# byuccl/coast

Hardware: NVIDIA H100
Metric: protected-kernel throughput (MB/s voted output), sha256 TMR (higher is better)
Workload: dtype u32

## Files before the change

coast_b200/csrc/xmr_aes128.cuh:

```cuda
#pragma once
#include "xmr_common.cuh"
#include "aes_tables.inc"

namespace xmr {

constexpr int AES_THREADS = XMR_AES_THREADS, AES_WARPS = XMR_AES_WARPS;
constexpr uint32_t AES_TAB01 = XMR_AES_TAB01, AES_TAB23 = XMR_AES_TAB23, AES_SIS = XMR_AES_SIS;
static_assert(AES_TAB01 + 256u * 64u * 4u <= AES_TAB23 && AES_TAB23 + 256u * 64u * 4u <= xmr_aes_smem(false) &&
              AES_SIS + 256u * 32u * 4u <= xmr_aes_smem(true), "the tables fit the launch's shared memory");
template <int NC> struct AesGeom {
    static constexpr int J = (int)xmr_aes_blocks_per_lane(NC);
    static constexpr int TROWS = AES_WARPS * Lanes<NC>::kUnitsPerWarp * J;
    static_assert(TROWS == xmr_aes_tile_rows(NC), "the host's tile");
};

constexpr int AES_STAGES = 3;
template <int TILE_ROWS>
struct AesRing {
    static constexpr int LOADS = (int)xmr_ring_loads(TILE_ROWS);
    static constexpr int BOX_ROWS = TILE_ROWS / LOADS;
    static constexpr uint32_t TILE_BYTES = (uint32_t)TILE_ROWS * 16u;
    static constexpr uint32_t STAGE_STRIDE = xmr_ring_stride(TILE_ROWS, 16u);
    static constexpr uint32_t SMEM_BYTES = xmr_ring_smem(AES_STAGES, TILE_ROWS, 16u, 128u);
    static_assert(2 * AES_STAGES * sizeof(uint64_t) <= 128u, "full and empty barriers fit behind the tiles");
    uint8_t* tiles; uint64_t* full; uint64_t* empty; const CUtensorMap* tmap; uint32_t pack_shift;
    __device__ __forceinline__ void init(uint8_t* smem, const CUtensorMap* map, uint32_t row_pack_shift) {
        tiles = smem; tmap = map; pack_shift = row_pack_shift;
        full = reinterpret_cast<uint64_t*>(smem + AES_STAGES * STAGE_STRIDE);
        empty = full + AES_STAGES;
        if (threadIdx.x == 0) {
            tma_prefetch_desc(map);
#pragma unroll
            for (int s = 0; s < AES_STAGES; ++s) { mbar_init(&full[s], 1); mbar_init(&empty[s], AES_WARPS); }
            fence_barrier_init();
        }
        __syncthreads();
    }
    __device__ __forceinline__ void issue(uint32_t it, uint32_t tile) {
        const uint32_t stage = it % AES_STAGES;
        mbar_arrive_expect_tx(&full[stage], TILE_BYTES);
#pragma unroll
        for (int l = 0; l < LOADS; ++l)
            tma_load_2d(tiles + stage * STAGE_STRIDE + l * BOX_ROWS * 16, tmap, &full[stage], 0, (int)((tile * TILE_ROWS + l * BOX_ROWS) >> pack_shift));
    }
    __device__ __forceinline__ const uint8_t* wait_full(uint32_t it) {
        mbar_wait(&full[it % AES_STAGES], (it / AES_STAGES) & 1u);
        return tiles + (it % AES_STAGES) * STAGE_STRIDE;
    }
    __device__ __forceinline__ void release(uint32_t it, int lane) {
        __syncwarp();
        if (lane == 0) asm volatile("mbarrier.arrive.shared::cta.b64 _, [%0];" ::"r"(smem_u32(&empty[it % AES_STAGES])) : "memory");
    }
    __device__ __forceinline__ void wait_empty(uint32_t it) {
        mbar_wait(&empty[it % AES_STAGES], (it / AES_STAGES) & 1u);
    }
};

__device__ __forceinline__ uint32_t lds32(uint32_t saddr) { uint32_t v; asm volatile("ld.shared.u32 %0, [%1];" : "=r"(v) : "r"(saddr)); return v; }
template <int K> __device__ __forceinline__ uint32_t tab(uint32_t lb, uint32_t t) { return lds32(__byte_perm(t, lb, 0x7604u | (K << 4))); }
template <int K> __device__ __forceinline__ uint32_t tab_half(uint32_t lb2x, uint32_t t) { return lds32(__byte_perm(t, lb2x, 0x7604u | (K << 4)) >> 1); }

__device__ __forceinline__ uint32_t xtime4(uint32_t w) { return ((w & 0x7F7F7F7Fu) << 1) ^ (((w >> 7) & 0x01010101u) * 0x1Bu); }
__device__ __forceinline__ uint32_t mix_column(uint32_t w) {
    const uint32_t r1 = __byte_perm(w, 0u, 0x0321u), r2 = __byte_perm(w, 0u, 0x1032u), r3 = __byte_perm(w, 0u, 0x2103u);
    return xtime4(w ^ r1) ^ r1 ^ r2 ^ r3;
}
__device__ __forceinline__ uint32_t inv_mix_column(uint32_t w) {
    const uint32_t v = w ^ __byte_perm(w, 0u, 0x1032u);
    return mix_column(w ^ xtime4(xtime4(v)));
}

struct AesLaneBases { uint32_t lb0, lb1, lb2, lb3, sis2x; };

template <bool DEC> __device__ __forceinline__ uint32_t sub_rot_word(const AesLaneBases& L, uint32_t w) {
    if (DEC) {
        const uint32_t a = tab_half<1>(L.sis2x, w), b = tab_half<2>(L.sis2x, w), c = tab_half<3>(L.sis2x, w), d = tab_half<0>(L.sis2x, w);
        return __byte_perm(__byte_perm(a, b, 0x0051u), __byte_perm(c, d, 0x0051u), 0x5410u);
    }
    return (tab<1>(L.lb2, w) & 0x000000FFu) | (tab<2>(L.lb0, w) & 0x0000FF00u) | (tab<3>(L.lb0, w) & 0x00FF0000u) | (tab<0>(L.lb1, w) & 0xFF000000u);
}
template <bool DEC> __device__ __forceinline__ void key_next(const AesLaneBases& L, uint32_t (&k)[4], int rd) {
    k[0] ^= sub_rot_word<DEC>(L, k[3]) ^ (uint32_t)XMR_AES_RCON[rd];
    k[1] ^= k[0]; k[2] ^= k[1]; k[3] ^= k[2];
}
template <bool DEC> __device__ __forceinline__ void key_prev(const AesLaneBases& L, uint32_t (&k)[4], int rd) {
    k[3] ^= k[2]; k[2] ^= k[1]; k[1] ^= k[0];
    k[0] ^= sub_rot_word<DEC>(L, k[3]) ^ (uint32_t)XMR_AES_RCON[rd];
}

template <bool DEC, bool LAST>
__device__ __forceinline__ void aes_round_cols(const AesLaneBases& L, const uint32_t (&t)[4], uint32_t (&n)[4]) {
    if (!DEC) {
        if (!LAST) {
#pragma unroll
            for (int c = 0; c < 4; ++c)
                n[c] = tab<0>(L.lb0, t[c]) ^ tab<1>(L.lb1, t[(c + 1) & 3]) ^ tab<2>(L.lb2, t[(c + 2) & 3]) ^ tab<3>(L.lb3, t[(c + 3) & 3]);
        } else {
#pragma unroll
            for (int c = 0; c < 4; ++c)
                n[c] = (tab<0>(L.lb2, t[c]) & 0x000000FFu) | (tab<1>(L.lb0, t[(c + 1) & 3]) & 0x0000FF00u) |
                       (tab<2>(L.lb0, t[(c + 2) & 3]) & 0x00FF0000u) | (tab<3>(L.lb1, t[(c + 3) & 3]) & 0xFF000000u);
        }
    } else {
        if (!LAST) {
#pragma unroll
            for (int c = 0; c < 4; ++c)
                n[c] = tab<0>(L.lb0, t[c]) ^ tab<1>(L.lb1, t[(c + 3) & 3]) ^ tab<2>(L.lb2, t[(c + 2) & 3]) ^ tab<3>(L.lb3, t[(c + 1) & 3]);
        } else {
#pragma unroll
            for (int c = 0; c < 4; ++c) {
                const uint32_t a = tab_half<0>(L.sis2x, t[c]), b = tab_half<1>(L.sis2x, t[(c + 3) & 3]);
                const uint32_t d = tab_half<2>(L.sis2x, t[(c + 2) & 3]), e = tab_half<3>(L.sis2x, t[(c + 1) & 3]);
                n[c] = __byte_perm(__byte_perm(a, b, 0x0040u), __byte_perm(d, e, 0x0040u), 0x5410u);
            }
        }
    }
}

template <int NC>
__device__ __forceinline__ void aes_vote_store(const uint32_t (&c)[4], uint8_t* out, unsigned long long local,
                                               unsigned long long gunit, bool valid, int lane, uint32_t flags, Tally& tally) {
    const bool majority = flags & COAST_F_MAJORITY_VOTER;
    uint32_t o[4], bad = 0;
#pragma unroll
    for (int i = 0; i < 4; ++i) { Voted v = vote_u32<NC, 1>(c[i], majority); o[i] = v.vote; bad += v.bad; }
    if (valid && Lanes<NC>::voter(lane)) {
        *reinterpret_cast<uint4*>(out + local * 16ull) = make_uint4(o[0], o[1], o[2], o[3]);
        tally.unit_exit<NC>(bad, 16u, flags, gunit);
    }
}

template <int J, bool DEC, bool PERKEY, bool HOOKS, bool ROLLED = false>
__device__ __forceinline__ void aes_rounds(const AesLaneBases& L, uint32_t (&s)[J][4], uint32_t (&k)[PERKEY ? J : 1][4], const uint32_t (&rk)[PERKEY ? 4 : 44],
                                           const uint32_t (&fbit)[J], const int (&frd)[J], const int (&fcol)[J]) {
    static_assert(!ROLLED || PERKEY, "a rolled round loop cannot index the register-resident round keys");
#pragma unroll (ROLLED ? 1 : 10)
    for (int rd = 0; rd < 10; ++rd) {
#pragma unroll
        for (int j = 0; j < J; ++j) {
            uint32_t n[4];
            if (rd < 9) aes_round_cols<DEC, false>(L, s[j], n); else aes_round_cols<DEC, true>(L, s[j], n);
            if (HOOKS) {
                uint32_t hit = frd[j] == rd ? fbit[j] : 0u;
                if (DEC && rd < 9) hit = inv_mix_column(hit);
#pragma unroll
                for (int c = 0; c < 4; ++c) n[c] ^= fcol[j] == c ? hit : 0u;
            }
            if (PERKEY) {
                if (!DEC) {
                    key_next<false>(L, k[j], rd);
#pragma unroll
                    for (int c = 0; c < 4; ++c) s[j][c] = n[c] ^ k[j][c];
                } else {
                    key_prev<true>(L, k[j], 9 - rd);
#pragma unroll
                    for (int c = 0; c < 4; ++c) s[j][c] = n[c] ^ (rd < 9 ? inv_mix_column(k[j][c]) : k[j][c]);
                }
            } else {
#pragma unroll
                for (int c = 0; c < 4; ++c) s[j][c] = n[c] ^ rk[4 * (rd + 1) + c];
            }
        }
    }
}

template <int J, bool DEC>
__device__ __forceinline__ void aes_rounds_hooked(const AesLaneBases& L, uint32_t (&s)[J][4], uint32_t rk_saddr,
                                               const uint32_t (&fbit)[J], const int (&frd)[J], const int (&fcol)[J]) {
#pragma unroll 1
    for (int rd = 0; rd < 10; ++rd) {
        uint32_t kr[4];
#pragma unroll
        for (int c = 0; c < 4; ++c) kr[c] = lds32(rk_saddr + 16u * (uint32_t)(rd + 1) + 4u * c);
#pragma unroll
        for (int j = 0; j < J; ++j) {
            uint32_t n[4];
            if (rd < 9) aes_round_cols<DEC, false>(L, s[j], n); else aes_round_cols<DEC, true>(L, s[j], n);
            uint32_t hit = frd[j] == rd ? fbit[j] : 0u;
            if (DEC && rd < 9) hit = inv_mix_column(hit);
#pragma unroll
            for (int c = 0; c < 4; ++c) s[j][c] = n[c] ^ (fcol[j] == c ? hit : 0u) ^ kr[c];
        }
    }
}

template <bool DEC>
__device__ __forceinline__ void aes_build_tables(uint8_t* smem_raw, uint32_t win, int tid) {
    uint32_t* t01 = reinterpret_cast<uint32_t*>(smem_raw + (AES_TAB01 - win));
    uint32_t* t23 = reinterpret_cast<uint32_t*>(smem_raw + (AES_TAB23 - win));
    for (int i = tid; i < 256 * 64; i += AES_THREADS) {
        uint32_t v;
        if (!DEC) v = XMR_AES_TE0[i >> 6];
        else v = inv_mix_column((uint32_t)XMR_AES_RSBOX[i >> 6]);
        const bool hi = (i & 32) != 0;
        t01[i] = hi ? __byte_perm(v, 0u, 0x2103u) : v;
        t23[i] = hi ? __byte_perm(v, 0u, 0x0321u) : __byte_perm(v, 0u, 0x1032u);
    }
    if (DEC) {
        uint32_t* sis = reinterpret_cast<uint32_t*>(smem_raw + (AES_SIS - win));
        for (int i = tid; i < 256 * 32; i += AES_THREADS) {
            const uint32_t is = XMR_AES_RSBOX[i >> 5], sb = XMR_AES_SBOX[i >> 5];
            sis[i] = is | (sb << 8) | (is << 16) | (sb << 24);
        }
    }
}
__device__ __forceinline__ AesLaneBases aes_lane_bases(int lane) {
    AesLaneBases L;
    L.lb0 = AES_TAB01 + 4u * lane; L.lb1 = AES_TAB01 + 128u + 4u * lane;
    L.lb2 = AES_TAB23 + 4u * lane; L.lb3 = AES_TAB23 + 128u + 4u * lane;
// ... 309 lines not shown
```

coast_b200/csrc/xmr_common.cuh:

```cuda
#pragma once
#include <cuda.h>
#include <cuda_runtime.h>
#include <stdint.h>
#include "../../include/coast_rt.h"
#include "xmr_args.h"
#include "xmr_geom.h"

namespace xmr {

struct u4 { uint32_t x, y, z, w; };

__device__ __forceinline__ u4 philox4x32_10(uint32_t c0, uint32_t c1, uint32_t c2, uint32_t c3, uint32_t k0, uint32_t k1) {
#pragma unroll
    for (int r = 0; r < 10; ++r) {
        uint32_t hi0 = __umulhi(0xD2511F53u, c0), lo0 = 0xD2511F53u * c0;
        uint32_t hi1 = __umulhi(0xCD9E8D57u, c2), lo1 = 0xCD9E8D57u * c2;
        uint32_t n0 = hi1 ^ c1 ^ k0, n2 = hi0 ^ c3 ^ k1;
        c0 = n0; c1 = lo1; c2 = n2; c3 = lo0;
        k0 += 0x9E3779B9u; k1 += 0xBB67AE85u;
    }
    return u4{c0, c1, c2, c3};
}

struct Fault { bool active; uint32_t replica, site, bit; };
// ... 72 lines not shown
    uint32_t e01 = eq_mask<EB>(x, r1), e02 = eq_mask<EB>(x, r2);
    v.vote = majority ? ((x & r1) | (x & r2) | (r1 & r2)) : ((x & e01) | (r2 & ~e01));
    v.bad = __popc(~(e01 & e02)) / (8 * EB);
    return v;
}

template <int NC>
__device__ __forceinline__ Voted vote_f32(float x, bool majority) {
    uint32_t xb = __float_as_uint(x);
    Voted v{xb, 0u};
    if (NC == 1) return v;
    float r1 = __shfl_down_sync(0xFFFFFFFFu, x, 1);
    if (NC == 2) { v.bad = (x == r1) ? 0u : 1u; return v; }
    float r2 = __shfl_down_sync(0xFFFFFFFFu, x, 2);
    bool c01 = (x == r1), c02 = (x == r2);
    uint32_t b1 = __float_as_uint(r1), b2 = __float_as_uint(r2);
    v.vote = majority ? ((xb & b1) | (xb & b2) | (b1 & b2)) : (c01 ? xb : b2);
    v.bad = (c01 && c02) ? 0u : 1u;
    return v;
}

template <int NC>
__device__ __forceinline__ uint32_t store_vote(uint32_t& x, int lane, bool majority) {
    if (NC == 1) return 0u;
    const int base = Lanes<NC>::unit(lane) * NC;
    const uint32_t r0 = __shfl_sync(0xFFFFFFFFu, x, base), r1 = __shfl_sync(0xFFFFFFFFu, x, base + 1);
    if (NC == 2) return r0 != r1 ? 1u : 0u;
    const uint32_t r2 = __shfl_sync(0xFFFFFFFFu, x, base + 2);
    const bool c01 = r0 == r1, c02 = r0 == r2;
    x = majority ? ((r0 & r1) | (r0 & r2) | (r1 & r2)) : (c01 ? r0 : r2);
    return (c01 && c02) ? 0u : 1u;
}

template <int NC>
__device__ __forceinline__ uint32_t store_vote_bytes(uint32_t& x, uint32_t nb, int lane, bool majority) {
    if (NC == 1 || nb == 0u) return 0u;
    const uint32_t live = 0xFFFFFFFFu << (8u * (4u - nb));
    const int base = Lanes<NC>::unit(lane) * NC;
    const uint32_t r0 = __shfl_sync(0xFFFFFFFFu, x, base), r1 = __shfl_sync(0xFFFFFFFFu, x, base + 1);
    const uint32_t e01 = __vcmpeq4(r0, r1);
    if (NC == 2) return __popc(~e01 & live) >> 3;
    const uint32_t r2 = __shfl_sync(0xFFFFFFFFu, x, base + 2);
    const uint32_t e02 = __vcmpeq4(r0, r2);
    x = majority ? ((r0 & r1) | (r0 & r2) | (r1 & r2)) : ((r0 & e01) | (r2 & ~e01));
    return __popc(~(e01 & e02) & live) >> 3;
}

struct Tally {
    uint32_t errors = 0, dwc = 0, syncs = 0, injected = 0;
    unsigned long long first = ~0ull;
    unsigned char* status = nullptr;
    unsigned long long base = 0;
    __device__ __forceinline__ Tally() {}
    __device__ __forceinline__ explicit Tally(const xmr_args& a) : status(a.status), base(a.unit_base) {}
    template <int NC> __device__ __forceinline__ void unit_exit(uint32_t bad, uint32_t nvotes, uint32_t flags, unsigned long long gunit) {
        if (NC == 3) {
            if (flags & COAST_F_COUNT_ERRORS) {
                errors += bad;
                if (flags & COAST_F_COUNT_SYNCS) syncs += nvotes;
            }
        } else if (NC == 2) {
            dwc += bad ? 1u : 0u;
        }
        if (NC > 1 && bad && gunit < first) first = gunit;
        if (status) status[gunit - base] = (unsigned char)(NC > 1 ? (bad > 255u ? 255u : bad) : 0u);
    }
    __device__ __forceinline__ void flush(unsigned long long* ctr) {
        uint32_t e = __reduce_add_sync(0xFFFFFFFFu, errors);
        uint32_t d = __reduce_add_sync(0xFFFFFFFFu, dwc);
        uint32_t s = __reduce_add_sync(0xFFFFFFFFu, syncs);
        uint32_t j = __reduce_add_sync(0xFFFFFFFFu, injected);
        uint32_t fhi = __reduce_min_sync(0xFFFFFFFFu, (uint32_t)(first >> 32));
        uint32_t flo = __reduce_min_sync(0xFFFFFFFFu, (uint32_t)(first >> 32) == fhi ? (uint32_t)first : 0xFFFFFFFFu);
        if ((threadIdx.x & 31) == 0) {
            if (e) atomicAdd_system(ctr + XMR_CTR_ERRORS, (unsigned long long)e);
            if (d) atomicAdd_system(ctr + XMR_CTR_DWC, (unsigned long long)d);
            if (s) atomicAdd_system(ctr + XMR_CTR_SYNCS, (unsigned long long)s);
            if (j) atomicAdd_system(ctr + XMR_CTR_INJECTED, (unsigned long long)j);
            unsigned long long f = ((unsigned long long)fhi << 32) | flo;
            if (f != ~0ull) atomicMin_system(ctr + XMR_CTR_FIRST, f);
        }
    }
};

__device__ __forceinline__ uint32_t smem_u32(const void* p) { return (uint32_t)__cvta_generic_to_shared(p); }

__device__ __forceinline__ void mbar_init(uint64_t* bar, uint32_t count) {
    asm volatile("mbarrier.init.shared::cta.b64 [%0], %1;" ::"r"(smem_u32(bar)), "r"(count));
}
__device__ __forceinline__ void fence_barrier_init() { asm volatile("fence.mbarrier_init.release.cluster;" ::: "memory"); }
__device__ __forceinline__ void fence_proxy_async() { asm volatile("fence.proxy.async.shared::cta;" ::: "memory"); }
__device__ __forceinline__ void mbar_arrive_expect_tx(uint64_t* bar, uint32_t bytes) {
    asm volatile("mbarrier.arrive.expect_tx.shared::cta.b64 _, [%0], %1;" ::"r"(smem_u32(bar)), "r"(bytes) : "memory");
}
__device__ __forceinline__ void mbar_wait(uint64_t* bar, uint32_t parity) {
    asm volatile(
        "{\n\t.reg .pred p;\n\t"
        "WAIT_%=:\n\t"
        "mbarrier.try_wait.parity.shared::cta.b64 p, [%0], %1;\n\t"
        "@p bra DONE_%=;\n\t"
        "bra WAIT_%=;\n\t"
        "DONE_%=:\n\t}" ::"r"(smem_u32(bar)), "r"(parity) : "memory");
}
__device__ __forceinline__ void tma_load_2d(void* smem_dst, const CUtensorMap* map, uint64_t* bar, int c0, int c1) {
    asm volatile(
        "cp.async.bulk.tensor.2d.shared::cluster.global.tile.mbarrier::complete_tx::bytes [%0], [%1, {%3, %4}], [%2];"
        ::"r"(smem_u32(smem_dst)), "l"(map), "r"(smem_u32(bar)), "r"(c0), "r"(c1) : "memory");
}
__device__ __forceinline__ void tma_prefetch_desc(const CUtensorMap* map) {
    asm volatile("prefetch.tensormap [%0];" ::"l"(map) : "memory");
}

template <int TILE_ROWS, int ROW_BYTES>
struct TileRing {
    static constexpr int LOADS = (int)xmr_ring_loads(TILE_ROWS);
    static constexpr int BOX_ROWS = TILE_ROWS / LOADS;
    static_assert(TILE_ROWS % LOADS == 0 && BOX_ROWS <= 256, "tile must split into equal TMA boxes");
    static constexpr uint32_t TILE_BYTES = (uint32_t)TILE_ROWS * ROW_BYTES;
    static constexpr uint32_t STAGE_STRIDE = xmr_ring_stride(TILE_ROWS, ROW_BYTES);
    static constexpr uint32_t SMEM_BYTES = xmr_ring_smem(XMR_STAGES, TILE_ROWS, ROW_BYTES, XMR_RING_TAIL);
    static_assert(XMR_STAGES * sizeof(uint64_t) <= XMR_RING_TAIL, "the full barriers fit behind the tiles");
    uint8_t* tiles;
    uint64_t* full;
    const CUtensorMap* tmap;
    uint32_t pack_shift = 0;
    __device__ __forceinline__ void init(uint8_t* smem, const CUtensorMap* map, uint32_t row_pack_shift = 0) {
        pack_shift = row_pack_shift;
        tiles = smem;
        full = reinterpret_cast<uint64_t*>(smem + XMR_STAGES * STAGE_STRIDE);
        tmap = map;
        if (threadIdx.x == 0) {
            tma_prefetch_desc(map);
#pragma unroll
            for (int s = 0; s < XMR_STAGES; ++s) mbar_init(&full[s], 1);
            fence_barrier_init();
        }
        __syncthreads();
    }
    __device__ __forceinline__ void issue(uint32_t stage, uint32_t tile) {
        if (threadIdx.x == 0) {
            mbar_arrive_expect_tx(&full[stage], TILE_BYTES);
#pragma unroll
            for (int l = 0; l < LOADS; ++l)
                tma_load_2d(tiles + stage * STAGE_STRIDE + l * BOX_ROWS * ROW_BYTES, tmap, &full[stage], 0,
                            (int)((tile * TILE_ROWS + l * BOX_ROWS) >> pack_shift));
        }
    }
    __device__ __forceinline__ const uint8_t* wait(uint32_t it) {
        mbar_wait(&full[it & 1u], (it >> 1) & 1u);
        return tiles + (it & 1u) * STAGE_STRIDE;
    }
};

}
```

coast_b200/csrc/xmr_geom.h:

```cpp
#ifndef XMR_GEOM_H_
#define XMR_GEOM_H_

#ifdef __CUDACC__
#define XMR_GEOM_FN static constexpr __host__ __device__ inline
#else
#define XMR_GEOM_FN static inline
#endif

XMR_GEOM_FN unsigned xmr_align(unsigned x, unsigned a) { return (x + a - 1u) & ~(a - 1u); }
XMR_GEOM_FN unsigned xmr_ring_stride(unsigned tile_rows, unsigned row_bytes) { return xmr_align(tile_rows * row_bytes, 1024u); }
XMR_GEOM_FN unsigned xmr_ring_smem(unsigned stages, unsigned tile_rows, unsigned row_bytes, unsigned tail) {
    return stages * xmr_ring_stride(tile_rows, row_bytes) + tail;
}
XMR_GEOM_FN unsigned xmr_ring_loads(unsigned tile_rows) {
    unsigned l = (tile_rows + 255u) / 256u;
    while (tile_rows % l) ++l;
    return l;
}
XMR_GEOM_FN unsigned xmr_units_per_warp(unsigned nc) { return 32u / nc; }

#define XMR_CTA_THREADS 256
#define XMR_WARPS       8
#define XMR_STAGES      2
#define XMR_RING_TAIL   64u
XMR_GEOM_FN unsigned xmr_sha_tile_rows(unsigned nc) { return XMR_WARPS * xmr_units_per_warp(nc); }
XMR_GEOM_FN unsigned xmr_sha_smem(unsigned nc) { return xmr_ring_smem(XMR_STAGES, xmr_sha_tile_rows(nc), 64u, XMR_RING_TAIL); }

#define XMR_SHA_SEG_THREADS    384
#define XMR_SHA_SEG_TILE_ROWS  128u
#define XMR_SHA_SEG_EXCH_BYTES (2u * 4u * 2u * 8u * 32u * 4u)
XMR_GEOM_FN unsigned xmr_sha_seg_exch_offset(void) {
    return xmr_align(xmr_ring_smem(XMR_STAGES, XMR_SHA_SEG_TILE_ROWS, 64u, XMR_RING_TAIL), 128u);
}
XMR_GEOM_FN unsigned xmr_sha_seg_smem(void) { return xmr_sha_seg_exch_offset() + XMR_SHA_SEG_EXCH_BYTES; }

#define XMR_CRC_TAB  0x10000u
#define XMR_CRC_RING 0x20000u
XMR_GEOM_FN unsigned xmr_crc_threads(unsigned nc) { return nc == 1u ? 768u : 1024u; }
XMR_GEOM_FN unsigned xmr_crc_tile_rows(unsigned nc) { return xmr_crc_threads(nc) / 32u * xmr_units_per_warp(nc); }
XMR_GEOM_FN unsigned xmr_crc_smem(unsigned nc) { return XMR_CRC_RING + xmr_ring_smem(XMR_STAGES, xmr_crc_tile_rows(nc), 64u, XMR_RING_TAIL); }

#define XMR_AES_THREADS 512
#define XMR_AES_WARPS   16
#define XMR_AES_TAB01   0x10000u
#define XMR_AES_TAB23   0x20000u
#define XMR_AES_SIS     0x30000u
XMR_GEOM_FN unsigned xmr_aes_blocks_per_lane(unsigned nc) { return nc == 1u ? 2u : 4u; }
XMR_GEOM_FN unsigned xmr_aes_tile_rows(unsigned nc) { return XMR_AES_WARPS * xmr_units_per_warp(nc) * xmr_aes_blocks_per_lane(nc); }
XMR_GEOM_FN unsigned xmr_aes_smem(int dec) { return dec ? XMR_AES_SIS + 0x8000u : XMR_AES_SIS; }

#define XMR_MMT_BM 64u
#define XMR_MMT_BN 128u
#define XMR_MMT_BK 16u
#define XMR_MMT_VT 128u
#define XMR_MMT_SMEM (64u * 1024u)
XMR_GEOM_FN unsigned xmr_mmt_threads(unsigned nc) { return nc * XMR_MMT_VT; }

#define XMR_WG_THREADS      384
#define XMR_WG_BM           128u
#define XMR_WG_SMEM_TAIL    (1024u + 256u)
#define XMR_PREPASS_THREADS 256
#define XMR_GEMM_BK 32u
XMR_GEOM_FN unsigned xmr_gemm_bn(int wide) { return wide ? 256u : 128u; }
XMR_GEOM_FN unsigned xmr_gemm_stages(int wide) { return wide ? 4u : 6u; }
XMR_GEOM_FN unsigned xmr_gemm_b_box(int pair) { return pair ? 64u : 128u; }
XMR_GEOM_FN unsigned xmr_gemm_smem(int wide) {
    return xmr_gemm_stages(wide) * (XMR_WG_BM * XMR_GEMM_BK * 4u + XMR_GEMM_BK * xmr_gemm_bn(wide) * 4u) + XMR_WG_SMEM_TAIL;
}
#define XMR_GEMM_BF16_BK    64u
#define XMR_GEMM_BF16_B_BOX 64u
#define XMR_MMTC_BK     128u
#define XMR_MMTC_STAGES 2u
XMR_GEOM_FN unsigned xmr_mmtc_bn(unsigned nc) { return nc == 1u ? 64u : 32u; }
XMR_GEOM_FN unsigned xmr_mmtc_smem(unsigned nc) {
    return XMR_MMTC_STAGES * (4u * XMR_WG_BM * XMR_MMTC_BK + 4u * xmr_mmtc_bn(nc) * XMR_MMTC_BK) + XMR_WG_SMEM_TAIL;
}

#define XMR_QSORT_THREADS 128

#define XMR_RAGGED_BUCKETS      1024u
#define XMR_RAGGED_HDR          64u
#define XMR_RAGGED_PERM         (XMR_RAGGED_HDR + 4u * XMR_RAGGED_BUCKETS)
#define XMR_RAGGED_SCAN_THREADS 1024
#define XMR_RAGGED_COST_CRC     0u
#define XMR_RAGGED_COST_SHA     1u
#define XMR_RAGGED_COST_QSORT   2u
XMR_GEOM_FN unsigned long long xmr_ragged_scratch(unsigned long long n_units) { return XMR_RAGGED_PERM + 4ull * n_units; }
XMR_GEOM_FN unsigned long long xmr_ragged_slots(unsigned long long n_units) { return (xmr_ragged_scratch(n_units) + 127ull) & ~127ull; }

#define XMR_MM_GRP_SCAN_THREADS 1024
#define XMR_MM_GRP_TILES        128u
#define XMR_MM_GRP_MAX          (1u << 20)
XMR_GEOM_FN unsigned long long xmr_mm_grp_bytes(unsigned long long groups) { return XMR_MM_GRP_TILES + 4ull * (groups + 1ull); }

#endif
```

coast_b200/csrc/xmr_sha256.cuh:

```cuda
#pragma once
#include "xmr_common.cuh"

namespace xmr {

__device__ __forceinline__ constexpr uint32_t sha_k(int i) {
    constexpr uint32_t K[64] = {
        0x428a2f98u, 0x71374491u, 0xb5c0fbcfu, 0xe9b5dba5u, 0x3956c25bu, 0x59f111f1u, 0x923f82a4u, 0xab1c5ed5u,
        0xd807aa98u, 0x12835b01u, 0x243185beu, 0x550c7dc3u, 0x72be5d74u, 0x80deb1feu, 0x9bdc06a7u, 0xc19bf174u,
        0xe49b69c1u, 0xefbe4786u, 0x0fc19dc6u, 0x240ca1ccu, 0x2de92c6fu, 0x4a7484aau, 0x5cb0a9dcu, 0x76f988dau,
        0x983e5152u, 0xa831c66du, 0xb00327c8u, 0xbf597fc7u, 0xc6e00bf3u, 0xd5a79147u, 0x06ca6351u, 0x14292967u,
        0x27b70a85u, 0x2e1b2138u, 0x4d2c6dfcu, 0x53380d13u, 0x650a7354u, 0x766a0abbu, 0x81c2c92eu, 0x92722c85u,
        0xa2bfe8a1u, 0xa81a664bu, 0xc24b8b70u, 0xc76c51a3u, 0xd192e819u, 0xd6990624u, 0xf40e3585u, 0x106aa070u,
        0x19a4c116u, 0x1e376c08u, 0x2748774cu, 0x34b0bcb5u, 0x391c0cb3u, 0x4ed8aa4au, 0x5b9cca4fu, 0x682e6ff3u,
        0x748f82eeu, 0x78a5636fu, 0x84c87814u, 0x8cc70208u, 0x90befffau, 0xa4506cebu, 0xbef9a3f7u, 0xc67178f2u};
    return K[i];
}

constexpr uint32_t SHA_SITES_PER_BLOCK = 536u;

__device__ __forceinline__ uint32_t rotr(uint32_t v, int n) { return __funnelshift_r(v, v, n); }
__device__ __forceinline__ uint32_t bswap(uint32_t v) { return __byte_perm(v, 0u, 0x0123u); }

__constant__ uint32_t sha_one = 1u;

__device__ __forceinline__ uint32_t add_imad(uint32_t x, uint32_t y) {
    uint32_t d;
    asm("mad.lo.u32 %0, %1, %2, %3;" : "=r"(d) : "r"(x), "r"(sha_one), "r"(y));
    return d;
}

template <bool INJECT, bool CONST_M = false>
__device__ __forceinline__ void sha_compress(uint32_t (&st)[8], uint32_t (&m)[16], uint32_t fs, uint32_t fmask) {
    if (INJECT && fs < 16u) {
#pragma unroll
        for (int i = 0; i < 16; ++i) m[i] ^= fs == (uint32_t)i ? fmask : 0u;
    }
    uint32_t a = st[0], b = st[1], c = st[2], d = st[3], e = st[4], f = st[5], g = st[6], h = st[7];
    const uint32_t ft = INJECT ? ((fs - 16u) >> 3) : 0u;
    const uint32_t fv = INJECT ? ((fs - 16u) & 7u) : 0u;
    const bool fround = INJECT && fs >= 16u && fs < 528u;
#pragma unroll
    for (int t = 0; t < 64; ++t) {
        if (t >= 16) {
            uint32_t w2 = m[(t - 2) & 15], w15 = m[(t - 15) & 15];
            uint32_t s1 = rotr(w2, 17) ^ rotr(w2, 19) ^ (w2 >> 10);
            uint32_t s0 = rotr(w15, 7) ^ rotr(w15, 18) ^ (w15 >> 3);
            m[t & 15] = CONST_M ? s1 + m[(t - 7) & 15] + s0 + m[t & 15]
                                : add_imad(s1, add_imad(s0, add_imad(m[(t - 7) & 15], m[t & 15])));
        }
        if (INJECT && fround && ft == (uint32_t)t) {
            a ^= fv == 0 ? fmask : 0u; b ^= fv == 1 ? fmask : 0u; c ^= fv == 2 ? fmask : 0u; d ^= fv == 3 ? fmask : 0u;
            e ^= fv == 4 ? fmask : 0u; f ^= fv == 5 ? fmask : 0u; g ^= fv == 6 ? fmask : 0u; h ^= fv == 7 ? fmask : 0u;
        }
        uint32_t ep0 = rotr(a, 2) ^ rotr(a, 13) ^ rotr(a, 22);
        uint32_t ep1 = rotr(e, 6) ^ rotr(e, 11) ^ rotr(e, 25);
        uint32_t ch = (e & f) ^ (~e & g);
        uint32_t maj = (a & b) ^ (a & c) ^ (b & c);
        uint32_t t1 = add_imad(ep1, add_imad(ch, add_imad(h, sha_k(t) + m[t & 15])));
        uint32_t t2 = add_imad(ep0, maj);
        h = g; g = f; f = e; e = add_imad(d, t1); d = c; c = b; b = a; a = add_imad(t1, t2);
    }
    st[0] += a; st[1] += b; st[2] += c; st[3] += d; st[4] += e; st[5] += f; st[6] += g; st[7] += h;
    if (INJECT && fs >= 528u && fs < 536u) {
#pragma unroll
        for (int i = 0; i < 8; ++i) st[i] ^= fs - 528u == (uint32_t)i ? fmask : 0u;
    }
}

template <int NC, bool INJECT>
__device__ __forceinline__ uint32_t sha_compress_sv(uint32_t (&st)[8], uint32_t (&m)[16], uint32_t fs, uint32_t fmask, int lane, bool majority) {
    uint32_t bad = 0;
#define SV(x) bad += store_vote<NC>(x, lane, majority)
#pragma unroll
    for (int i = 0; i < 16; ++i) { SV(m[i]); if (INJECT) m[i] ^= fs == (uint32_t)i ? fmask : 0u; }
    uint32_t v[8];
#pragma unroll
    for (int i = 0; i < 8; ++i) { v[i] = st[i]; SV(v[i]); }
    uint32_t a = v[0], b = v[1], c = v[2], d = v[3], e = v[4], f = v[5], g = v[6], h = v[7];
    const uint32_t ft = INJECT ? ((fs - 16u) >> 3) : 0u, fv = INJECT ? ((fs - 16u) & 7u) : 0u;
    const bool fround = INJECT && fs >= 16u && fs < 528u;
#pragma unroll 1
    for (int t = 0; t < 64; ++t) {
        if (t >= 16) {
            const uint32_t w2 = m[(t - 2) & 15], w15 = m[(t - 15) & 15];
            uint32_t w = (rotr(w2, 17) ^ rotr(w2, 19) ^ (w2 >> 10)) + m[(t - 7) & 15] + (rotr(w15, 7) ^ rotr(w15, 18) ^ (w15 >> 3)) + m[t & 15];
            SV(w);
            m[t & 15] = w;
        }
        if (INJECT && fround && ft == (uint32_t)t) {
            a ^= fv == 0 ? fmask : 0u; b ^= fv == 1 ? fmask : 0u; c ^= fv == 2 ? fmask : 0u; d ^= fv == 3 ? fmask : 0u;
            e ^= fv == 4 ? fmask : 0u; f ^= fv == 5 ? fmask : 0u; g ^= fv == 6 ? fmask : 0u; h ^= fv == 7 ? fmask : 0u;
        }
        uint32_t t1 = h + (rotr(e, 6) ^ rotr(e, 11) ^ rotr(e, 25)) + ((e & f) ^ (~e & g)) + sha_k(t) + m[t & 15];
        SV(t1);
        uint32_t t2 = (rotr(a, 2) ^ rotr(a, 13) ^ rotr(a, 22)) + ((a & b) ^ (a & c) ^ (b & c));
        SV(t2);
        uint32_t x;
        x = g; SV(x); h = x;
        x = f; SV(x); g = x;
        x = e; SV(x); f = x;
        x = d + t1; SV(x); e = x;
        x = c; SV(x); d = x;
        x = b; SV(x); c = x;
        x = a; SV(x); b = x;
        x = t1 + t2; SV(x); a = x;
    }
    const uint32_t add[8] = {a, b, c, d, e, f, g, h};
#pragma unroll
    for (int i = 0; i < 8; ++i) {
        uint32_t x = st[i] + add[i];
        SV(x);
        st[i] = x;
        if (INJECT) st[i] ^= (fs >= 528u && fs - 528u == (uint32_t)i) ? fmask : 0u;
    }
#undef SV
    return bad;
}

__device__ __forceinline__ void sha_init(uint32_t (&st)[8]) {
    st[0] = 0x6a09e667u; st[1] = 0xbb67ae85u; st[2] = 0x3c6ef372u; st[3] = 0xa54ff53au;
    st[4] = 0x510e527fu; st[5] = 0x9b05688cu; st[6] = 0x1f83d9abu; st[7] = 0x5be0cd19u;
}

template <int NC>
__device__ __forceinline__ void sha_vote_store(const uint32_t (&st)[8], uint8_t* out, unsigned long long local,
                                               unsigned long long gunit, bool valid, int lane, uint32_t flags, Tally& tally) {
    const bool majority = flags & COAST_F_MAJORITY_VOTER;
    uint32_t o[8], bad = 0;
#pragma unroll
    for (int i = 0; i < 8; ++i) {
        Voted v = vote_u32<NC, 1>(st[i], majority);
        o[i] = bswap(v.vote);
        bad += v.bad;
    }
    if (valid && Lanes<NC>::voter(lane)) {
        uint4* dst = reinterpret_cast<uint4*>(out + local * 32ull);
        dst[0] = make_uint4(o[0], o[1], o[2], o[3]);
        dst[1] = make_uint4(o[4], o[5], o[6], o[7]);
        tally.unit_exit<NC>(bad, 32u, flags, gunit);
    }
}

template <int NC, bool INJECT>
__device__ __forceinline__ void sha256_b64_body(const xmr_args& a, const CUtensorMap* tmap) {
    constexpr int UPW = Lanes<NC>::kUnitsPerWarp;
    constexpr int TU = XMR_WARPS * UPW;
    static_assert(TU == xmr_sha_tile_rows(NC) && TileRing<TU, 64>::SMEM_BYTES <= xmr_sha_smem(NC), "ring fits the launch's shared memory");
    extern __shared__ __align__(1024) uint8_t smem_raw[];
    TileRing<TU, 64> ring;
    ring.init(smem_raw, tmap);

    const int tid = threadIdx.x, lane = tid & 31, warp = tid >> 5;
    const int r = Lanes<NC>::replica(lane);
    const int ul = warp * UPW + Lanes<NC>::unit(lane);

    const uint32_t n_tiles = a.n_tiles;
    uint32_t tile = blockIdx.x;
    if (tile < n_tiles) ring.issue(0, tile);
    Tally tally(a);
    uint32_t it = 0;
    for (; tile < n_tiles; tile += gridDim.x, ++it) {
        const uint32_t next = tile + gridDim.x;
        if (next < n_tiles) ring.issue((it + 1u) & 1u, next);
        const uint8_t* base = ring.wait(it);

        uint32_t m[16];
        const uint8_t* row = base + ul * 64;
        const int sw = (ul >> 1) & 3;
#pragma unroll
        for (int c = 0; c < 4; ++c) {
            uint4 q = *reinterpret_cast<const uint4*>(row + ((c ^ sw) << 4));
            m[4 * c + 0] = bswap(q.x); m[4 * c + 1] = bswap(q.y); m[4 * c + 2] = bswap(q.z); m[4 * c + 3] = bswap(q.w);
        }
        __syncthreads();

        const unsigned long long local = (unsigned long long)tile * TU + ul;
        const bool valid = local < a.n_units;
        const unsigned long long gunit = a.unit_base + local;

        uint32_t fs0 = 0xFFFFFFFFu, fs1 = 0xFFFFFFFFu, fmask = 0u;
        if (INJECT) {
            Fault f = fault_for_unit(a, NC, valid ? local : 0ull, [](uint32_t) { return 32u; });
            if (f.active && valid) {
                if (Lanes<NC>::voter(lane)) tally.injected++;
                if ((int)f.replica == r) {
                    fmask = 1u << f.bit;
                    if (f.site < SHA_SITES_PER_BLOCK) fs0 = f.site; else fs1 = f.site - SHA_SITES_PER_BLOCK;
                }
            }
        }

        uint32_t st[8];
        sha_init(st);
        sha_compress<INJECT>(st, m, fs0, fmask);
#pragma unroll
        for (int i = 0; i < 16; ++i) m[i] = 0u;
        m[0] = 0x80000000u; m[15] = 512u;
        sha_compress<INJECT, true>(st, m, fs1, fmask);

        sha_vote_store<NC>(st, static_cast<uint8_t*>(a.out), local, gunit, valid, lane, a.flags, tally);
    }
    tally.flush(a.counters);
}

__device__ __forceinline__ uint32_t sha_padded_byte(const uint8_t* msg, uint32_t len, uint32_t pos) {
    return pos < len ? (uint32_t)__ldg(msg + pos) : (pos == len ? 0x80u : 0u);
}

template <int NC, bool INJECT>
__device__ __forceinline__ void sha256_gen_body(const xmr_args& a) {
    constexpr int UPW = Lanes<NC>::kUnitsPerWarp;
    const int lane = threadIdx.x & 31;
    const int r = Lanes<NC>::replica(lane);
    const unsigned long long gwarp = ((unsigned long long)blockIdx.x * blockDim.x + threadIdx.x) >> 5;
    const unsigned long long nwarps = ((unsigned long long)gridDim.x * blockDim.x) >> 5;
    const uint32_t len = a.unit_bytes;
    const uint32_t nblk = (len + 8u) / 64u + 1u;
    const unsigned long long n_wtiles = (a.n_units + UPW - 1) / UPW;
    Tally tally(a);
    for (unsigned long long wt = gwarp; wt < n_wtiles; wt += nwarps) {
        const unsigned long long local = wt * UPW + Lanes<NC>::unit(lane);
        const bool valid = local < a.n_units;
        const unsigned long long gunit = a.unit_base + local;
        const uint8_t* msg = static_cast<const uint8_t*>(a.in) + (valid ? local : 0ull) * len;
        uint32_t fsite = 0xFFFFFFFFu, fmask = 0u;
        if (INJECT) {
            Fault f = fault_for_unit(a, NC, valid ? local : 0ull, [](uint32_t) { return 32u; });
            if (f.active && valid) {
                if (Lanes<NC>::voter(lane)) tally.injected++;
                if ((int)f.replica == r) { fmask = 1u << f.bit; fsite = f.site; }
            }
        }
        const bool sv = (a.flags & XMR_F_STORE_VOTES) != 0;
        const bool majority = a.flags & COAST_F_MAJORITY_VOTER;
        uint32_t sv_bad = 0;
        uint32_t st[8];
        sha_init(st);
        const uintptr_t al = reinterpret_cast<uintptr_t>(a.in) | len;
        for (uint32_t blk = 0; blk < nblk; ++blk) {
            uint32_t m[16];
            if ((al & 15u) == 0 && blk * 64u + 64u <= len) {
#pragma unroll
                for (int c = 0; c < 4; ++c) {
                    const uint4 q = __ldg(reinterpret_cast<const uint4*>(msg + blk * 64u) + c);
                    m[4 * c + 0] = bswap(q.x); m[4 * c + 1] = bswap(q.y); m[4 * c + 2] = bswap(q.z); m[4 * c + 3] = bswap(q.w);
                }
            } else {
#pragma unroll
                for (int w = 0; w < 16; ++w) {
                    const uint32_t p = blk * 64u + 4u * w;
                    if ((al & 3u) == 0 && p + 4u <= len) m[w] = bswap(__ldg(reinterpret_cast<const uint32_t*>(msg + p)));
                    else m[w] = (sha_padded_byte(msg, len, p) << 24) | (sha_padded_byte(msg, len, p + 1) << 16) |
                                (sha_padded_byte(msg, len, p + 2) << 8) | sha_padded_byte(msg, len, p + 3);
                }
            }
            if (blk == nblk - 1) {
                m[14] = len >> 29;
                m[15] = len << 3;
            }
            uint32_t fs = (INJECT && fsite / SHA_SITES_PER_BLOCK == blk) ? fsite % SHA_SITES_PER_BLOCK : 0xFFFFFFFFu;
            if (!sv) {
                sha_compress<INJECT>(st, m, fs, fmask);
            } else {
                const uint32_t lo = blk * 64u, nmsg = len > lo ? (len - lo < 64u ? len - lo : 64u) : 0u;
#pragma unroll
                for (int w = 0; w < 16; ++w) {
                    const uint32_t nb = nmsg > 4u * w ? (nmsg - 4u * w < 4u ? nmsg - 4u * w : 4u) : 0u;
                    sv_bad += store_vote_bytes<NC>(m[w], nb, lane, majority);
                }
                sv_bad += sha_compress_sv<NC, INJECT>(st, m, fs, fmask, lane, majority);
            }
        }
        if (!sv) {
            sha_vote_store<NC>(st, static_cast<uint8_t*>(a.out), local, gunit, valid, lane, a.flags, tally);
        } else {
            uint32_t o[8], bad = 0;
#pragma unroll
            for (int i = 0; i < 8; ++i) { Voted v = vote_u32<NC, 1>(st[i], majority); o[i] = bswap(v.vote); bad += v.bad; }
            if (valid && Lanes<NC>::voter(lane)) {
                uint4* dst = reinterpret_cast<uint4*>(static_cast<uint8_t*>(a.out) + local * 32ull);
                dst[0] = make_uint4(o[0], o[1], o[2], o[3]);
                dst[1] = make_uint4(o[4], o[5], o[6], o[7]);
                tally.unit_exit<NC>(bad + sv_bad, len + 720u * nblk + 32u, a.flags, gunit);
            }
        }
    }
    tally.flush(a.counters);
}

constexpr int SEG_THREADS = XMR_SHA_SEG_THREADS, SEG_GROUPS = SEG_THREADS / 96, SEG_TU = SEG_GROUPS * 32;
constexpr uint32_t SEG_EXCH_WORDS = 2 * 8 * 32;

template <bool INJECT>
__device__ __forceinline__ void sha256_b64_seg_body(const xmr_args& a, const CUtensorMap* tmap) {
    using Ring = TileRing<SEG_TU, 64>;
    static_assert(SEG_TU == XMR_SHA_SEG_TILE_ROWS && Ring::SMEM_BYTES <= xmr_sha_seg_exch_offset() &&
                  xmr_sha_seg_exch_offset() + 2u * SEG_GROUPS * SEG_EXCH_WORDS * 4u <= xmr_sha_seg_smem(),
                  "ring and exchange buffer fit the launch's shared memory");
    extern __shared__ __align__(1024) uint8_t smem_raw[];
    Ring ring;
    ring.init(smem_raw, tmap);
    uint32_t* exch = reinterpret_cast<uint32_t*>(smem_raw + xmr_sha_seg_exch_offset());
    const int tid = threadIdx.x, lane = tid & 31, warp = tid >> 5;
    const int g = warp / 3, r = warp - 3 * g;
    const int ul = g * 32 + lane;
    const uint32_t n_tiles = a.n_tiles;
    const bool majority = a.flags & COAST_F_MAJORITY_VOTER;
    uint32_t tile = blockIdx.x;
    if (tile < n_tiles) ring.issue(0, tile);
    Tally tally(a);
    uint32_t it = 0;
    for (; tile < n_tiles; tile += gridDim.x, ++it) {
        const uint32_t next = tile + gridDim.x;
        if (next < n_tiles) ring.issue((it + 1u) & 1u, next);
        const uint8_t* base = ring.wait(it);
        uint32_t m[16];
        const uint8_t* row = base + ul * 64;
        const int sw = (ul >> 1) & 3;
#pragma unroll
        for (int c = 0; c < 4; ++c) {
            uint4 q = *reinterpret_cast<const uint4*>(row + ((c ^ sw) << 4));
            m[4 * c + 0] = bswap(q.x); m[4 * c + 1] = bswap(q.y); m[4 * c + 2] = bswap(q.z); m[4 * c + 3] = bswap(q.w);
        }
        __syncthreads();
        const unsigned long long local = (unsigned long long)tile * SEG_TU + ul;
        const bool valid = local < a.n_units;
        uint32_t fs0 = 0xFFFFFFFFu, fs1 = 0xFFFFFFFFu, fmask = 0u;
        if (INJECT) {
            Fault f = fault_for_unit(a, 3, valid ? local : 0ull, [](uint32_t) { return 32u; });
            if (f.active && valid) {
                if (r == 0) tally.injected++;
                if ((int)f.replica == r) {
                    fmask = 1u << f.bit;
                    if (f.site < SHA_SITES_PER_BLOCK) fs0 = f.site; else fs1 = f.site - SHA_SITES_PER_BLOCK;
                }
            }
        }
        uint32_t st[8];
        sha_init(st);
        sha_compress<INJECT>(st, m, fs0, fmask);
#pragma unroll
        for (int i = 0; i < 16; ++i) m[i] = 0u;
        m[0] = 0x80000000u; m[15] = 512u;
        sha_compress<INJECT, true>(st, m, fs1, fmask);

        uint32_t* ex = exch + ((it & 1u) * SEG_GROUPS + g) * SEG_EXCH_WORDS;
        if (r > 0) {
#pragma unroll
            for (int i = 0; i < 8; ++i) ex[((r - 1) * 8 + i) * 32 + lane] = st[i];
        }
        if (g == 0) asm volatile("bar.sync 1, 96;" ::: "memory");
        else if (g == 1) asm volatile("bar.sync 2, 96;" ::: "memory");
        else if (g == 2) asm volatile("bar.sync 3, 96;" ::: "memory");
        else asm volatile("bar.sync 4, 96;" ::: "memory");
        if (r == 0) {
            uint32_t o[8], bad = 0;
#pragma unroll
            for (int i = 0; i < 8; ++i) {
                const uint32_t x = st[i], r1 = ex[i * 32 + lane], r2 = ex[(8 + i) * 32 + lane];
                const uint32_t e01 = __vcmpeq4(x, r1), e02 = __vcmpeq4(x, r2);
                const uint32_t v = majority ? ((x & r1) | (x & r2) | (r1 & r2)) : ((x & e01) | (r2 & ~e01));
                bad += __popc(~(e01 & e02)) >> 3;
                o[i] = bswap(v);
            }
            if (valid) {
                uint4* dst = reinterpret_cast<uint4*>(static_cast<uint8_t*>(a.out) + local * 32ull);
                dst[0] = make_uint4(o[0], o[1], o[2], o[3]);
                dst[1] = make_uint4(o[4], o[5], o[6], o[7]);
                tally.unit_exit<3>(bad, 32u, a.flags, a.unit_base + local);
            }
        }
    }
    tally.flush(a.counters);
}

}

#define XMR_SHA_B64_KERNEL(NC, INJ)                                                                      \
    extern "C" __global__ void __launch_bounds__(XMR_CTA_THREADS)                                        \
    xmr_sha256_b64_nc##NC##_inj##INJ(const __grid_constant__ xmr_args a, const __grid_constant__ CUtensorMap tmap) { \
        xmr::sha256_b64_body<NC, INJ != 0>(a, &tmap);                                                    \
    }
#define XMR_SHA_GEN_KERNEL(NC, INJ)                                                                      \
    extern "C" __global__ void __launch_bounds__(XMR_CTA_THREADS)                                        \
    xmr_sha256_gen_nc##NC##_inj##INJ(const __grid_constant__ xmr_args a) {                               \
        xmr::sha256_gen_body<NC, INJ != 0>(a);                                                           \
    }
XMR_SHA_B64_KERNEL(1, 0) XMR_SHA_B64_KERNEL(2, 0) XMR_SHA_B64_KERNEL(3, 0)
XMR_SHA_B64_KERNEL(1, 1) XMR_SHA_B64_KERNEL(2, 1) XMR_SHA_B64_KERNEL(3, 1)
XMR_SHA_GEN_KERNEL(1, 0) XMR_SHA_GEN_KERNEL(2, 0) XMR_SHA_GEN_KERNEL(3, 0)
XMR_SHA_GEN_KERNEL(1, 1) XMR_SHA_GEN_KERNEL(2, 1) XMR_SHA_GEN_KERNEL(3, 1)

#define XMR_SHA_B64_SEG_KERNEL(INJ)                                                                      \
    extern "C" __global__ void __launch_bounds__(xmr::SEG_THREADS)                                       \
    xmr_sha256_b64_seg_nc3_inj##INJ(const __grid_constant__ xmr_args a, const __grid_constant__ CUtensorMap tmap) { \
        xmr::sha256_b64_seg_body<INJ != 0>(a, &tmap);                                                    \
    }
XMR_SHA_B64_SEG_KERNEL(0) XMR_SHA_B64_SEG_KERNEL(1)
```

Measured before the change: 84410.

## Deepen SHA seg TMA ring with mbarrier release and fast-path voter

Replaces the two-stage ring in the segmented SHA-256 TMR kernel with a generic four-stage mbarrier ring. Tiles are prefetched two ahead, and each warp releases its stage through an empty barrier instead of a CTA-wide __syncthreads. The voter first checks with a single lop3 whether the three replicas differ at all and only does the per-byte compare and majority work when they do. Launch bounds now request 2 or 3 CTAs per SM, which caps registers and may cause spills. The extra stages use more shared memory, which may limit occupancy.

Result: faster. 86320, median of 6 (+2.3%).

```diff
diff --git a/coast_b200/csrc/xmr_aes128.cuh b/coast_b200/csrc/xmr_aes128.cuh
--- a/coast_b200/csrc/xmr_aes128.cuh
+++ b/coast_b200/csrc/xmr_aes128.cuh
@@ -16,45 +16,7 @@
 
 constexpr int AES_STAGES = 3;
 template <int TILE_ROWS>
-struct AesRing {
-    static constexpr int LOADS = (int)xmr_ring_loads(TILE_ROWS);
-    static constexpr int BOX_ROWS = TILE_ROWS / LOADS;
-    static constexpr uint32_t TILE_BYTES = (uint32_t)TILE_ROWS * 16u;
-    static constexpr uint32_t STAGE_STRIDE = xmr_ring_stride(TILE_ROWS, 16u);
-    static constexpr uint32_t SMEM_BYTES = xmr_ring_smem(AES_STAGES, TILE_ROWS, 16u, 128u);
-    static_assert(2 * AES_STAGES * sizeof(uint64_t) <= 128u, "full and empty barriers fit behind the tiles");
-    uint8_t* tiles; uint64_t* full; uint64_t* empty; const CUtensorMap* tmap; uint32_t pack_shift;
-    __device__ __forceinline__ void init(uint8_t* smem, const CUtensorMap* map, uint32_t row_pack_shift) {
-        tiles = smem; tmap = map; pack_shift = row_pack_shift;
-        full = reinterpret_cast<uint64_t*>(smem + AES_STAGES * STAGE_STRIDE);
-        empty = full + AES_STAGES;
-        if (threadIdx.x == 0) {
-            tma_prefetch_desc(map);
-#pragma unroll
-            for (int s = 0; s < AES_STAGES; ++s) { mbar_init(&full[s], 1); mbar_init(&empty[s], AES_WARPS); }
-            fence_barrier_init();
-        }
-        __syncthreads();
-    }
-    __device__ __forceinline__ void issue(uint32_t it, uint32_t tile) {
-        const uint32_t stage = it % AES_STAGES;
-        mbar_arrive_expect_tx(&full[stage], TILE_BYTES);
-#pragma unroll
-        for (int l = 0; l < LOADS; ++l)
-            tma_load_2d(tiles + stage * STAGE_STRIDE + l * BOX_ROWS * 16, tmap, &full[stage], 0, (int)((tile * TILE_ROWS + l * BOX_ROWS) >> pack_shift));
-    }
-    __device__ __forceinline__ const uint8_t* wait_full(uint32_t it) {
-        mbar_wait(&full[it % AES_STAGES], (it / AES_STAGES) & 1u);
-        return tiles + (it % AES_STAGES) * STAGE_STRIDE;
-    }
-    __device__ __forceinline__ void release(uint32_t it, int lane) {
-        __syncwarp();
-        if (lane == 0) asm volatile("mbarrier.arrive.shared::cta.b64 _, [%0];" ::"r"(smem_u32(&empty[it % AES_STAGES])) : "memory");
-    }
-    __device__ __forceinline__ void wait_empty(uint32_t it) {
-        mbar_wait(&empty[it % AES_STAGES], (it / AES_STAGES) & 1u);
-    }
-};
+using AesRing = MbarRing<TILE_ROWS, 16, AES_STAGES, AES_WARPS>;
 
 __device__ __forceinline__ uint32_t lds32(uint32_t saddr) { uint32_t v; asm volatile("ld.shared.u32 %0, [%1];" : "=r"(v) : "r"(saddr)); return v; }
 template <int K> __device__ __forceinline__ uint32_t tab(uint32_t lb, uint32_t t) { return lds32(__byte_perm(t, lb, 0x7604u | (K << 4))); }
diff --git a/coast_b200/csrc/xmr_common.cuh b/coast_b200/csrc/xmr_common.cuh
--- a/coast_b200/csrc/xmr_common.cuh
+++ b/coast_b200/csrc/xmr_common.cuh
@@ -248,4 +248,47 @@
     }
 };
 
-}
+template <int TILE_ROWS, int ROW_BYTES, int STAGES, int WARPS>
+struct MbarRing {
+    static constexpr int LOADS = (int)xmr_ring_loads(TILE_ROWS);
+    static constexpr int BOX_ROWS = TILE_ROWS / LOADS;
+    static_assert(TILE_ROWS % LOADS == 0 && BOX_ROWS <= 256, "tile must split into equal TMA boxes");
+    static constexpr uint32_t TILE_BYTES = (uint32_t)TILE_ROWS * ROW_BYTES;
+    static constexpr uint32_t STAGE_STRIDE = xmr_ring_stride(TILE_ROWS, ROW_BYTES);
+    static constexpr uint32_t SMEM_BYTES = xmr_ring_smem(STAGES, TILE_ROWS, ROW_BYTES, XMR_MBAR_RING_TAIL);
+    static_assert(2 * STAGES * sizeof(uint64_t) <= XMR_MBAR_RING_TAIL, "full and empty barriers fit behind the tiles");
+    uint8_t* tiles; uint64_t* full; uint64_t* empty; const CUtensorMap* tmap; uint32_t pack_shift;
+    __device__ __forceinline__ void init(uint8_t* smem, const CUtensorMap* map, uint32_t row_pack_shift = 0) {
+        tiles = smem; tmap = map; pack_shift = row_pack_shift;
+        full = reinterpret_cast<uint64_t*>(smem + STAGES * STAGE_STRIDE);
+        empty = full + STAGES;
+        if (threadIdx.x == 0) {
+            tma_prefetch_desc(map);
+#pragma unroll
+            for (int s = 0; s < STAGES; ++s) { mbar_init(&full[s], 1); mbar_init(&empty[s], WARPS); }
+            fence_barrier_init();
+        }
+        __syncthreads();
+    }
+    __device__ __forceinline__ void issue(uint32_t it, uint32_t tile) {
+        const uint32_t stage = it % STAGES;
+        mbar_arrive_expect_tx(&full[stage], TILE_BYTES);
+#pragma unroll
+        for (int l = 0; l < LOADS; ++l)
+            tma_load_2d(tiles + stage * STAGE_STRIDE + l * BOX_ROWS * ROW_BYTES, tmap, &full[stage], 0,
+                        (int)((tile * TILE_ROWS + l * BOX_ROWS) >> pack_shift));
+    }
+    __device__ __forceinline__ const uint8_t* wait_full(uint32_t it) {
+        mbar_wait(&full[it % STAGES], (it / STAGES) & 1u);
+        return tiles + (it % STAGES) * STAGE_STRIDE;
+    }
+    __device__ __forceinline__ void release(uint32_t it, int lane) {
+        __syncwarp();
+        if (lane == 0) asm volatile("mbarrier.arrive.shared::cta.b64 _, [%0];" ::"r"(smem_u32(&empty[it % STAGES])) : "memory");
+    }
+    __device__ __forceinline__ void wait_empty(uint32_t it) {
+        mbar_wait(&empty[it % STAGES], (it / STAGES) & 1u);
+    }
+};
+
+}
diff --git a/coast_b200/csrc/xmr_geom.h b/coast_b200/csrc/xmr_geom.h
--- a/coast_b200/csrc/xmr_geom.h
+++ b/coast_b200/csrc/xmr_geom.h
@@ -23,14 +23,16 @@
 #define XMR_WARPS       8
 #define XMR_STAGES      2
 #define XMR_RING_TAIL   64u
+#define XMR_MBAR_RING_TAIL 128u
 XMR_GEOM_FN unsigned xmr_sha_tile_rows(unsigned nc) { return XMR_WARPS * xmr_units_per_warp(nc); }
 XMR_GEOM_FN unsigned xmr_sha_smem(unsigned nc) { return xmr_ring_smem(XMR_STAGES, xmr_sha_tile_rows(nc), 64u, XMR_RING_TAIL); }
 
 #define XMR_SHA_SEG_THREADS    384
 #define XMR_SHA_SEG_TILE_ROWS  128u
+#define XMR_SHA_SEG_STAGES     4
 #define XMR_SHA_SEG_EXCH_BYTES (2u * 4u * 2u * 8u * 32u * 4u)
 XMR_GEOM_FN unsigned xmr_sha_seg_exch_offset(void) {
-    return xmr_align(xmr_ring_smem(XMR_STAGES, XMR_SHA_SEG_TILE_ROWS, 64u, XMR_RING_TAIL), 128u);
+    return xmr_align(xmr_ring_smem(XMR_SHA_SEG_STAGES, XMR_SHA_SEG_TILE_ROWS, 64u, XMR_MBAR_RING_TAIL), 128u);
 }
 XMR_GEOM_FN unsigned xmr_sha_seg_smem(void) { return xmr_sha_seg_exch_offset() + XMR_SHA_SEG_EXCH_BYTES; }
 
diff --git a/coast_b200/csrc/xmr_sha256.cuh b/coast_b200/csrc/xmr_sha256.cuh
--- a/coast_b200/csrc/xmr_sha256.cuh
+++ b/coast_b200/csrc/xmr_sha256.cuh
@@ -20,6 +20,11 @@
 
 __device__ __forceinline__ uint32_t rotr(uint32_t v, int n) { return __funnelshift_r(v, v, n); }
 __device__ __forceinline__ uint32_t bswap(uint32_t v) { return __byte_perm(v, 0u, 0x0123u); }
+__device__ __forceinline__ uint32_t differs3(uint32_t x, uint32_t y, uint32_t z) {
+    uint32_t d;
+    asm("lop3.b32 %0, %1, %2, %3, 0x7e;" : "=r"(d) : "r"(x), "r"(y), "r"(z));
+    return d;
+}
 
 __constant__ uint32_t sha_one = 1u;
 
@@ -289,11 +294,14 @@
 }
 
 constexpr int SEG_THREADS = XMR_SHA_SEG_THREADS, SEG_GROUPS = SEG_THREADS / 96, SEG_TU = SEG_GROUPS * 32;
+constexpr int SEG_STAGES = XMR_SHA_SEG_STAGES;
+constexpr uint32_t SEG_AHEAD = 2;
 constexpr uint32_t SEG_EXCH_WORDS = 2 * 8 * 32;
 
 template <bool INJECT>
 __device__ __forceinline__ void sha256_b64_seg_body(const xmr_args& a, const CUtensorMap* tmap) {
-    using Ring = TileRing<SEG_TU, 64>;
+    using Ring = MbarRing<SEG_TU, 64, SEG_STAGES, SEG_THREADS / 32>;
+    static_assert(SEG_AHEAD >= 1 && SEG_AHEAD < (uint32_t)SEG_STAGES, "a refill never waits on the tile being read");
     static_assert(SEG_TU == XMR_SHA_SEG_TILE_ROWS && Ring::SMEM_BYTES <= xmr_sha_seg_exch_offset() &&
                   xmr_sha_seg_exch_offset() + 2u * SEG_GROUPS * SEG_EXCH_WORDS * 4u <= xmr_sha_seg_smem(),
                   "ring and exchange buffer fit the launch's shared memory");
@@ -307,13 +315,15 @@
     const uint32_t n_tiles = a.n_tiles;
     const bool majority = a.flags & COAST_F_MAJORITY_VOTER;
     uint32_t tile = blockIdx.x;
-    if (tile < n_tiles) ring.issue(0, tile);
+    if (tid == 0) {
+#pragma unroll
+        for (uint32_t i = 0; i < SEG_AHEAD; ++i)
+            if (tile + i * gridDim.x < n_tiles) ring.issue(i, tile + i * gridDim.x);
+    }
     Tally tally(a);
     uint32_t it = 0;
     for (; tile < n_tiles; tile += gridDim.x, ++it) {
-        const uint32_t next = tile + gridDim.x;
-        if (next < n_tiles) ring.issue((it + 1u) & 1u, next);
-        const uint8_t* base = ring.wait(it);
+        const uint8_t* base = ring.wait_full(it);
         uint32_t m[16];
         const uint8_t* row = base + ul * 64;
         const int sw = (ul >> 1) & 3;
@@ -322,7 +332,14 @@
             uint4 q = *reinterpret_cast<const uint4*>(row + ((c ^ sw) << 4));
             m[4 * c + 0] = bswap(q.x); m[4 * c + 1] = bswap(q.y); m[4 * c + 2] = bswap(q.z); m[4 * c + 3] = bswap(q.w);
         }
-        __syncthreads();
+        ring.release(it, lane);
+        if (tid == 0) {
+            const uint32_t ahead = tile + SEG_AHEAD * gridDim.x;
+            if (ahead < n_tiles) {
+                if (it + SEG_AHEAD >= (uint32_t)SEG_STAGES) ring.wait_empty(it + SEG_AHEAD - SEG_STAGES);
+                ring.issue(it + SEG_AHEAD, ahead);
+            }
+        }
         const unsigned long long local = (unsigned long long)tile * SEG_TU + ul;
         const bool valid = local < a.n_units;
         uint32_t fs0 = 0xFFFFFFFFu, fs1 = 0xFFFFFFFFu, fmask = 0u;
@@ -354,15 +371,24 @@
         else if (g == 2) asm volatile("bar.sync 3, 96;" ::: "memory");
         else asm volatile("bar.sync 4, 96;" ::: "memory");
         if (r == 0) {
-            uint32_t o[8], bad = 0;
+            uint32_t r1[8], r2[8], v[8], o[8], bad = 0, diff = 0;
 #pragma unroll
             for (int i = 0; i < 8; ++i) {
-                const uint32_t x = st[i], r1 = ex[i * 32 + lane], r2 = ex[(8 + i) * 32 + lane];
-                const uint32_t e01 = __vcmpeq4(x, r1), e02 = __vcmpeq4(x, r2);
-                const uint32_t v = majority ? ((x & r1) | (x & r2) | (r1 & r2)) : ((x & e01) | (r2 & ~e01));
-                bad += __popc(~(e01 & e02)) >> 3;
-                o[i] = bswap(v);
-            }
+                r1[i] = ex[i * 32 + lane]; r2[i] = ex[(8 + i) * 32 + lane];
+                diff |= differs3(st[i], r1[i], r2[i]);
+                v[i] = st[i];
+            }
+            if (__builtin_expect(diff != 0u, 0)) {
+#pragma unroll
+                for (int i = 0; i < 8; ++i) {
+                    const uint32_t x = st[i];
+                    const uint32_t e01 = __vcmpeq4(x, r1[i]), e02 = __vcmpeq4(x, r2[i]);
+                    v[i] = majority ? ((x & r1[i]) | (x & r2[i]) | (r1[i] & r2[i])) : ((x & e01) | (r2[i] & ~e01));
+                    bad += __popc(~(e01 & e02)) >> 3;
+                }
+            }
+#pragma unroll
+            for (int i = 0; i < 8; ++i) o[i] = bswap(v[i]);
             if (valid) {
                 uint4* dst = reinterpret_cast<uint4*>(static_cast<uint8_t*>(a.out) + local * 32ull);
                 dst[0] = make_uint4(o[0], o[1], o[2], o[3]);
@@ -392,7 +418,7 @@
 XMR_SHA_GEN_KERNEL(1, 1) XMR_SHA_GEN_KERNEL(2, 1) XMR_SHA_GEN_KERNEL(3, 1)
 
 #define XMR_SHA_B64_SEG_KERNEL(INJ)                                                                      \
-    extern "C" __global__ void __launch_bounds__(xmr::SEG_THREADS)                                       \
+    extern "C" __global__ void __launch_bounds__(xmr::SEG_THREADS, (INJ) ? 2 : 3)                        \
     xmr_sha256_b64_seg_nc3_inj##INJ(const __grid_constant__ xmr_args a, const __grid_constant__ CUtensorMap tmap) { \
         xmr::sha256_b64_seg_body<INJ != 0>(a, &tmap);                                                    \
     }
```
